# liayan/Legion-1

Hardware: AMD Instinct MI355X
Metric: sampled edges/s + feature GB/s, 3-hop GraphSAGE ogbn-papers100M at 1/2/4/8 GPU (higher is better)
Workload: dtype int32 ids / f32 rows (verbatim copy)

## Files before the change

### legion-1_amd/csrc/internal.h

```cpp
#pragma once
#include <hip/hip_runtime.h>
#include <cstdint>
#include <cstdio>
#include <cstdlib>
#include <iostream>
#include <string>
#include <vector>

#include "../../include/legion_amd.h"
#include "audit.h"

namespace legion {

void report_error(const char* file, int line, const char* msg, bool hip_failure);
bool error_pending();
bool error_is_fatal();
int64_t ipc_max_bytes();
bool ipc_size_ok(int64_t bytes, const char* who);
bool ipc_export_ok(const void* ptr, const char* who);
int64_t shard_chunk_bytes();
inline void check(hipError_t e, const char* file, int line)
{
    if (e != hipSuccess) report_error(file, line, hipGetErrorString(e), true);
}
#define HIP_CHECK(expr) ::legion::check((expr), __FILE__, __LINE__)
#define HIP_CHECK_LAST() ::legion::check(hipGetLastError(), __FILE__, __LINE__)
#define LEGION_ARG_ERROR(msg) ::legion::report_error(__FILE__, __LINE__, (msg), false)

std::ostream& log_out();
FILE* log_file();

int physical_device(int logical);
bool is_remote_device(int logical);
struct DeviceGuard {
    int prev = -1, prev_logical = -1;
    explicit DeviceGuard(int logical);
    ~DeviceGuard();
};

int chunk_shift(int64_t unit_bytes, int min_shift);
inline int chunk_count(int64_t n, int shift) { return n > 0 ? (int)(((n - 1) >> shift) + 1) : 1; }
template <typename T>
struct ChunkList {
    std::vector<T*> chunks;
    bool imported = false;
    T* at(int q) const { return q >= 0 && q < (int)chunks.size() ? chunks[q] : nullptr; }
    bool complete(size_t n) const { for (T* p : chunks) if (!p) return false; return chunks.size() == n; }
    void release();
    int export_chunk(int dev, int q, void* handle64, const char* who) const;
    int import_chunk(int q, const void* handle64, int64_t floor_bytes, int open_dev, const char* who);
};
template <typename T> void upload_table(int viewer, const std::vector<T*>& h, T**& tab, bool realloc, const char* what);

typedef unsigned long long pos_t;
constexpr int kPosShift = 32;
constexpr uint32_t kProvisional = 0x80000000u, kPosValueMask = 0x7FFFFFFFu;
constexpr uint32_t kEpochTop = 0xFFFFFFFFu, kSerialLimit = 0xFFFFFFF0u;
__host__ __device__ inline pos_t pos_entry(uint32_t epoch, uint32_t value) { return ((pos_t)epoch << kPosShift) | (pos_t)value; }
#ifndef LEGION_KTILE
#define LEGION_KTILE 1024
#endif
constexpr int kTile = LEGION_KTILE;
constexpr int kBlock = 256;
static_assert(kTile >= kBlock && kTile <= 2048 && (kTile & (kTile - 1)) == 0, "LEGION_KTILE: a power of two in [256, 2048] (k_sample stages 16 bytes of row descriptor per slot in static LDS)");
constexpr int kMaxChunks = 2048;
static_assert(kMaxChunks % kBlock == 0 && kMaxChunks >= 256 * 8, "kMaxChunks: a multiple of the workgroup size, >= 256 CUs x 8 workgroups");
constexpr int ilog2_c(int v) { return v <= 1 ? 0 : 1 + ilog2_c(v >> 1); }
constexpr int kMaxParts = LEGION_MAX_DEVICE;

constexpr uint32_t kP31 = 2147483647u;
constexpr uint32_t kA = 48271u;

__host__ __device__ inline uint32_t mulmod31(uint32_t a, uint32_t b)
{
    uint64_t p = (uint64_t)a * (uint64_t)b;
    uint32_t r = (uint32_t)(p & kP31) + (uint32_t)(p >> 31);
    r = (r & kP31) + (r >> 31);
    return r >= kP31 ? r - kP31 : r;
}

__host__ __device__ inline uint32_t powmod31(uint32_t base, uint64_t e)
{
    uint32_t r = 1;
    while (e) {
        if (e & 1) r = mulmod31(r, base);
        base = mulmod31(base, base);
        e >>= 1;
    }
    return r;
}

struct FastDiv {
    uint32_t d = 1, m = 0, s = 0;
    FastDiv() = default;
    explicit FastDiv(uint32_t div);
};

struct CsrTables {
    const int64_t* indptr;
    const int32_t* indices;
    const int64_t* const* frag_indptr;
    const int32_t* const* frag_indices;
    int32_t ip_nch, ix_nch, row_shift, edge_shift;
    int32_t partition_count;
    const int8_t* topo_owner;
    const int32_t* topo_row;
};

struct BatchCtl {
    int32_t counter;
    uint32_t epoch;
};

struct HopState {
    int32_t edge_base, node_base, n_edges, n_nodes, in_off, n_in, slots, pad;
};

struct SamplerBuffers {
    int32_t* sampled_ids;
    int32_t* agg_src_ids;
    int32_t* agg_src_off;
    int32_t* agg_dst_off;
    int32_t* nc;
    int32_t* ec;
    pos_t* pos_map;
    const BatchCtl* ctl;
    int32_t* cand;
    int32_t* aux;
    int32_t* aux_next;
    int32_t next_count;
    int32_t aux_cap;
    int32_t ids_cap;
    int32_t V;
    bool aux_prepared;
    int32_t* tile_edge;
    int32_t* tile_node;
    int2* tile_pre;
    int2* chunk_tot;
    HopState* hop_state;
    unsigned long long* edge_access_time;
};

void launch_seed(hipStream_t s, int32_t* batch_ids, int32_t* labels, int32_t batch_size, int32_t size, int32_t counter,
                 const int32_t* all_ids, const int32_t* all_labels, int32_t total_cap, pos_t* pos_map,
                 uint32_t epoch, BatchCtl* ctl, bool self_driven, int32_t* nc, int32_t* ec, int32_t* aux_next,
                 int32_t f_next, int32_t aux_cap);
void launch_set_cursor(hipStream_t s, BatchCtl* ctl, int32_t counter, uint32_t epoch);
void launch_advance(hipStream_t s, BatchCtl* ctl);
void warm_static_tables();
void launch_sample_hop(hipStream_t s, const CsrTables& csr, const SamplerBuffers& b, int32_t count, int32_t op_id,
                       int32_t hops, int32_t slots_bound, bool is_presc);
void launch_find_feat(hipStream_t s, const int32_t* sampled_ids, int32_t* cache_offset, const int32_t* nc,
                      int32_t op_id, const int32_t* feat_map, int32_t bound);
void launch_find_topo(hipStream_t s, const int32_t* input_ids, int8_t* part_index, int32_t* part_offset,
                      int32_t batch_size, const int8_t* topo_owner, const int32_t* topo_row);
struct GatherArgs {
    const float* table;
    const float* const* shard_tab;
    int32_t chunk_shift, nchunks;
    const int32_t* feat_map;
    const float** row_ptr;
    int32_t cache_capacity;
    int32_t F;
    int32_t table_pitch, shard_pitch;
    int32_t total_num_nodes;
    const int32_t* sampled_ids;
    const int32_t* nc;
    float* dst;
// ... 156 lines not shown
```

### legion-1_amd/csrc/kernels.hip

```cpp
#include "internal.h"
#include <hipcub/hipcub.hpp>
#include <mutex>
#include <cstring>

#include "audit_hooks.h"

namespace legion {

__device__ inline int32_t sample_index(uint32_t x, int32_t deg)
{
    double result = (double)(uint32_t)(x - 1u);
    result /= 2147483646.0;
    return (int32_t)(result * (double)deg + 0.0);
}

__device__ inline uint32_t fdiv(uint32_t n, const FastDiv& d)
{
    return d.d == 1 ? n : (uint32_t)(((uint64_t)n * d.m) >> d.s);
}

__device__ inline int lane_id() { return threadIdx.x & 63; }
__device__ inline int wave_id() { return threadIdx.x >> 6; }

__device__ inline int32_t total_nodes(const int32_t* nc, int32_t hops) { return nc[5 + 2 * hops]; }

template <bool SELF>
__global__ __launch_bounds__(kBlock) void k_seed(int32_t* __restrict__ batch_ids, int32_t* __restrict__ labels,
                                                 int32_t batch_size, int32_t size, int32_t counter,
                                                 const int32_t* __restrict__ all_ids,
                                                 const int32_t* __restrict__ all_labels, int32_t total_cap,
                                                 pos_t* __restrict__ pos_map, uint32_t epoch,
                                                 BatchCtl* __restrict__ ctl, int32_t* __restrict__ nc,
                                                 int32_t* __restrict__ ec, int32_t* __restrict__ aux_next,
                                                 int32_t f_next, int32_t aux_cap)
{
    int32_t idx = threadIdx.x + blockDim.x * blockIdx.x;
    if (SELF) {
        counter = ctl->counter;
        epoch = ctl->epoch;
        const int64_t done = (int64_t)batch_size * counter;
        size = (done + batch_size >= total_cap) ? (int32_t)max((int64_t)0, min((int64_t)batch_size, (int64_t)total_cap - done)) : batch_size;
    } else if (idx == 0) {
        ctl->counter = counter;
        ctl->epoch = epoch;
    }
    if (idx < size) {
        int32_t g = size * counter + idx;
        if (g >= total_cap) {
            batch_ids[idx] = -1;
            labels[idx] = -1;
        } else {
            int32_t src_id = all_ids[g % total_cap];
            batch_ids[idx] = src_id;
            const pos_t mine = pos_entry(epoch, (uint32_t)idx);
            pos_t cur = pos_map[src_id];
            while ((uint32_t)(cur >> kPosShift) != epoch || cur < mine) {
                const pos_t seen = atomicCAS(pos_map + src_id, cur, mine);
                if (seen == cur) break;
                cur = seen;
            }
            labels[idx] = all_labels[g % total_cap];
        }
    }
    if (idx < 16) {
        int32_t nv = 0;
        if (idx == 0 || idx == 2 || idx == 4) nv = size;
        nc[idx] = nv;
        ec[idx] = 0;
    }
    const int64_t n_init = min((int64_t)max(size, 0) * f_next, (int64_t)aux_cap);
    for (int64_t i = idx; i < n_init; i += (int64_t)gridDim.x * blockDim.x) aux_next[i] = -1;
}
__global__ void k_fill_aux(const int32_t* __restrict__ nc, int32_t count, int32_t* __restrict__ aux, int32_t aux_cap)
{
    const int64_t n = min((int64_t)nc[2] * count, (int64_t)aux_cap);
    for (int64_t i = threadIdx.x + (int64_t)blockDim.x * blockIdx.x; i < n; i += (int64_t)gridDim.x * blockDim.x) aux[i] = -1;
}
__global__ void k_set_cursor(BatchCtl* ctl, int32_t counter, uint32_t epoch) { ctl->counter = counter; ctl->epoch = epoch; }
__global__ void k_advance(BatchCtl* ctl) { ctl->counter += 1; ctl->epoch -= 1; }


struct SampleArgs {
    CsrTables csr;
    const int32_t* sampled_ids;
    const int32_t* agg_src_ids;
    const int32_t* nc;
    const int32_t* ec;
    pos_t* pos_map;
    int32_t* cand;
    int32_t* aux;
    int32_t* tile_edge;
    unsigned long long* edge_access_time;
    const BatchCtl* ctl;
    const uint32_t* pow_tab;
    uint32_t a_tile;
    uint32_t a_step;
    FastDiv fdiv;
    int32_t count;
    int32_t op_id;
    int32_t window;
    int32_t prefilter_from_op;
};

__device__ inline int32_t claim_slot(const SampleArgs& a, uint32_t epoch, int32_t dst, int32_t idx)
{
    const pos_t prov0 = pos_entry(epoch, kProvisional);
    const pos_t mine = prov0 | (pos_t)(uint32_t)idx;
    pos_t cur = (a.op_id < a.prefilter_from_op) ? ~(pos_t)0 : a.pos_map[dst];
    if (cur > mine) {
        const pos_t old = atomicMin(a.pos_map + dst, mine);
        if (old > mine) {
            if ((uint32_t)(old >> kPosShift) == epoch) a.aux[(uint32_t)old & kPosValueMask] = -2 - idx;
            cur = mine;
        } else {
            cur = old;
        }
    }
    if (cur < prov0) return (int32_t)((uint32_t)cur & kPosValueMask);
    if (cur < mine) return -2 - (int32_t)((uint32_t)cur & kPosValueMask);
    return -1;
}

template <bool PRESC, bool PARTITIONED>
__global__ __launch_bounds__(kBlock) void k_sample(SampleArgs a)
{
    __shared__ const int32_t* s_row[kTile + 2];
    __shared__ int32_t s_deg[kTile + 2];
    __shared__ int32_t s_src[kTile + 2];
    __shared__ int32_t s_cnt[kBlock / 64];

    const int32_t N = a.nc[2];
    const int32_t f = a.count;
    const int32_t total = N * f;
    const int32_t* __restrict__ input = (a.op_id == 2) ? a.sampled_ids : a.agg_src_ids + a.ec[2];
    const int32_t n_tiles = (total + kTile - 1) / kTile;
    const int tid = threadIdx.x;
    const uint32_t epoch = a.ctl->epoch;

    if ((int32_t)blockIdx.x >= n_tiles) return;

    uint32_t x[kTile / kBlock];
    {
        uint32_t base = powmod31(a.a_tile, (uint64_t)blockIdx.x);
#pragma unroll
        for (int s = 0; s < kTile / kBlock; s++) x[s] = mulmod31(base, a.pow_tab[tid + kBlock * s]);
    }

    for (int32_t tile = blockIdx.x; tile < n_tiles; tile += gridDim.x) {
        const int32_t tile_start = tile * kTile;
        const int32_t tile_end = min(tile_start + kTile, total);
        const int32_t i0 = (int32_t)fdiv((uint32_t)tile_start, a.fdiv);
        const int32_t i_last = (int32_t)fdiv((uint32_t)(tile_end - 1), a.fdiv);
        const int32_t nrows = i_last - i0 + 1;

        for (int32_t r = tid; r < nrows; r += kBlock) {
            const int32_t src = input[i0 + r];
            const int32_t* rowp = nullptr;
            int32_t deg = -1;
            if (src >= 0) {
                const int64_t* ip = a.csr.indptr + src;
                const int32_t* ix = a.csr.indices;
                int8_t owner = -1;
                if (PARTITIONED && !PRESC) owner = a.csr.topo_owner[src];
                if (owner >= 0) {
                    const int32_t row = a.csr.topo_row[src];
                    ip = a.csr.frag_indptr[owner * a.csr.ip_nch + (row >> a.csr.row_shift)] + (row & ((1 << a.csr.row_shift) - 1));
                    const int64_t start = ip[0];
                    ix = a.csr.frag_indices[owner * a.csr.ix_nch + (int32_t)(start >> a.csr.edge_shift)];
                    rowp = ix + (start & ((1ll << a.csr.edge_shift) - 1));
                    deg = (int32_t)(ip[1] - start);
                } else {
                    const int64_t start = ip[0];
                    rowp = ix + start;
                    deg = (int32_t)(ip[1] - start);
                }
            }
            s_row[r] = rowp;
            s_deg[r] = deg;
            s_src[r] = src;
        }
        __syncthreads();

        int32_t cnt = 0;
#pragma unroll
        for (int s = 0; s < kTile / kBlock; s++) {
            const int32_t idx = tile_start + tid + kBlock * s;
            int32_t dst = -1, known = -1, j = 0, r = 0;
            if (idx < tile_end) {
                const uint32_t i = fdiv((uint32_t)idx, a.fdiv);
                j = idx - (int32_t)i * f;
                r = (int32_t)i - i0;
                const int32_t deg = s_deg[r];
                if (j < deg) {
                    dst = s_row[r][sample_index(x[s], deg)];
                    if (dst < 0) dst = -1;
                }
            }
            int32_t dup = 0;
            for (int d = 1; d <= a.window; d++) {
                const int32_t o = __shfl_up(dst, d);
                if (d <= j && d <= lane_id() && o == dst) dup = d;
            }
            if (dst >= 0) {
                if (PRESC) atomicAdd(a.edge_access_time + s_src[r], 1ull);
                if (dup) known = -2 - (idx - dup);
                else known = claim_slot(a, epoch, dst, idx);
                cnt++;
            }
            if (idx < tile_end) {
                a.cand[idx] = dst;
                if (dst < 0) a.aux[idx] = 0;
                else if (known != -1) a.aux[idx] = known;
            }
        }
        for (int o = 32; o > 0; o >>= 1) cnt += __shfl_down(cnt, o);
        if (lane_id() == 0) s_cnt[wave_id()] = cnt;
        __syncthreads();
        if (tid == 0) {
            int32_t t = 0;
#pragma unroll
            for (int w = 0; w < kBlock / 64; w++) t += s_cnt[w];
            a.tile_edge[tile] = t;
        }
#pragma unroll
        for (int s = 0; s < kTile / kBlock; s++) x[s] = mulmod31(x[s], a.a_step);
        __syncthreads();
    }
}

constexpr int32_t kWinBase = 0x40000000;

__device__ inline int32_t enc_win(int32_t r) { return -2 - (kWinBase + r); }
__device__ inline bool is_win(int32_t v) { return v <= -2 - kWinBase; }
__device__ inline int32_t win_rank(int32_t v) { return -2 - v - kWinBase; }

__host__ __device__ inline FastDiv make_fastdiv(uint32_t div)
{
    FastDiv f;
    f.d = div ? div : 1;
    if (f.d == 1) { f.m = 0; f.s = 0; return f; }
    uint32_t l = 0;
    while ((1ull << l) < f.d) l++;
    f.m = (uint32_t)(((1ull << (31 + l)) / f.d) + 1ull);
    f.s = 31 + l;
    return f;
}

__global__ __launch_bounds__(kBlock) void k_mark(const int32_t* __restrict__ nc, const int32_t* __restrict__ ec,
                                                 int32_t count, int32_t* __restrict__ aux, const int32_t* __restrict__ tile_edge,
                                                 int32_t* __restrict__ tile_node, int2* __restrict__ tile_pre,
                                                 int2* __restrict__ chunk_tot, HopState* __restrict__ hs)
{
    constexpr int S = kTile / kBlock, W = kBlock / 64;
    __shared__ int32_t s_c[S * W];
    const int32_t total = nc[2] * count;
    const int32_t n_tiles = (total + kTile - 1) / kTile;
    const int lane = lane_id(), wave = wave_id();
    const unsigned long long lt = (1ull << lane) - 1ull;
    if (blockIdx.x == 0 && threadIdx.x == 0) {
        HopState h;
        h.edge_base = ec[0]; h.node_base = nc[0]; h.n_edges = 0; h.n_nodes = 0;
        h.in_off = ec[2]; h.n_in = nc[2]; h.slots = total; h.pad = 0;
        *hs = h;
    }
    const int32_t T = (n_tiles + (int32_t)gridDim.x - 1) / (int32_t)gridDim.x;
    const int32_t t0 = (int32_t)blockIdx.x * T, t1 = min(t0 + T, n_tiles);
    if (t0 >= n_tiles) return;
    int32_t nxt[S];
#pragma unroll
    for (int s = 0; s < S; s++) {
        const int64_t idx = (int64_t)t0 * kTile + threadIdx.x + kBlock * s;
        nxt[s] = idx < total ? aux[idx] : 0;
    }
    int32_t te_next = threadIdx.x == 0 ? tile_edge[t0] : 0, run_e = 0, run_n = 0;
    for (int32_t tile = t0; tile < t1; tile++) {
        bool win[S];
        int32_t rk[S];
        const int32_t te = te_next;
#pragma unroll
        for (int s = 0; s < S; s++) {
            const int32_t idx = tile * kTile + threadIdx.x + kBlock * s;
            win[s] = idx < total && nxt[s] == -1;
        }
        {
            const int64_t nt = (int64_t)tile + 1;
#pragma unroll
            for (int s = 0; s < S; s++) {
                const int64_t idx = nt * kTile + threadIdx.x + kBlock * s;
                nxt[s] = (nt < t1 && idx < total) ? aux[idx] : 0;
            }
            if (threadIdx.x == 0 && nt < t1) te_next = tile_edge[nt];
        }
#pragma unroll
        for (int s = 0; s < S; s++) {
            const unsigned long long b = __ballot(win[s]);
            rk[s] = __popcll(b & lt);
            if (lane == 0) s_c[s * W + wave] = __popcll(b);
        }
        __syncthreads();
        int32_t run = 0, before[S];
#pragma unroll
        for (int q = 0; q < S * W; q++) {
#pragma unroll
            for (int s = 0; s < S; s++)
                if (q == s * W + wave) before[s] = run;
            run += s_c[q];
        }
#pragma unroll
        for (int s = 0; s < S; s++)
            if (win[s]) aux[tile * kTile + threadIdx.x + kBlock * s] = enc_win(before[s] + rk[s]);
        if (threadIdx.x == 0) {
            tile_node[tile] = run;
            tile_pre[tile] = make_int2(run_e, run_n);
            run_e += te; run_n += run;
        }
        __syncthreads();
    }
    if (threadIdx.x == 0) chunk_tot[blockIdx.x] = make_int2(run_e, run_n);
}

__device__ inline void apply_update_counter(int32_t* nc, int32_t* ec, int32_t op_id, int32_t hops, int32_t n_nodes,
                                            int32_t n_edges)
{
    const int32_t hh = op_id / 2;
    nc[0] += n_nodes;
    nc[3 + 2 * hh] = nc[1 + 2 * hh] + nc[2 + 2 * hh];
    nc[4 + 2 * hh] = n_nodes;
    if (hh == hops) nc[5 + 2 * hh] = nc[3 + 2 * hh] + nc[4 + 2 * hh];
    nc[1] = 0;
    nc[2] = n_edges;
    ec[2 + hh] = (hh == 1 ? ec[3] : ec[1 + hh]) + n_edges;
    ec[2] = ec[0];
    ec[0] += n_edges;
    ec[1] = 0;
}

struct WriteArgs {
    HopState* hs;
    int32_t* nc;
    int32_t* ec;
    int32_t hops;
    const int32_t* cand;
    const int32_t* aux;
    const int32_t* tile_edge;
    const int32_t* tile_node;
    int32_t* sampled_ids;
    int32_t* agg_src_ids;
    int32_t* agg_src_off;
    int32_t* agg_dst_off;
    pos_t* pos_map;
    FastDiv fdiv;
    int32_t op_id;
    const BatchCtl* ctl;
    int32_t last_hop;
    const int2* tile_pre;
    const int2* chunk_tot;
    int32_t mark_grid;
    int32_t* aux_next;
    int32_t next_count;
    int32_t aux_cap;
    int32_t ids_cap;
    int32_t V;
};

#define LEGION_STORE_OK(i, cap) ((uint32_t)(i) < (uint32_t)(cap))

__global__ __launch_bounds__(kBlock) void k_write(WriteArgs a)
{
    constexpr int S = kTile / kBlock, W = kBlock / 64;
    __shared__ int2 s_chunk[kMaxChunks];
    __shared__ int32_t s_e[S * W];
    __shared__ int2 s_scan[W];
    __shared__ uint32_t s_div_t[3];
    const HopState h = *a.hs;
    const uint32_t epoch = a.ctl->epoch;
    const int32_t total = h.slots;
    const int32_t n_tiles = (total + kTile - 1) / kTile;
    const int lane = lane_id(), wave = wave_id();
    const unsigned long long lt = (1ull << lane) - 1ull;
    if (n_tiles == 0) {
        if (blockIdx.x == 0 && threadIdx.x == 0) apply_update_counter(a.nc, a.ec, a.op_id, a.hops, 0, 0);
        return;
    }
    if ((int32_t)blockIdx.x >= n_tiles) return;
    const int32_t T = (n_tiles + a.mark_grid - 1) / a.mark_grid;
    if (threadIdx.x == 0) {
        const FastDiv f = make_fastdiv((uint32_t)T);
        s_div_t[0] = f.d; s_div_t[1] = f.m; s_div_t[2] = f.s;
    }
    const int32_t n_chunks = (n_tiles + T - 1) / T;
    {
        constexpr int PER = kMaxChunks / kBlock;
        const int32_t q0 = (int32_t)threadIdx.x * PER;
        int2 v[PER];
#pragma unroll
        for (int u = 0; u < PER; u++) v[u] = a.chunk_tot[min(q0 + u, n_chunks - 1)];
        int32_t se = 0, sn = 0;
#pragma unroll
        for (int u = 0; u < PER; u++) {
            if (q0 + u >= n_chunks) v[u] = make_int2(0, 0);
            se += v[u].x; sn += v[u].y;
        }
        int32_t ie = se, in = sn;
        for (int o = 1; o < 64; o <<= 1) {
            const int32_t ue = __shfl_up(ie, o), un = __shfl_up(in, o);
            if (lane >= o) { ie += ue; in += un; }
        }
        if (lane == 63) s_scan[wave] = make_int2(ie, in);
// ... 3 lines not shown
        for (int w = 0; w < W; w++)
            if (w < wave) { run_e += s_scan[w].x; run_n += s_scan[w].y; }
#pragma unroll
        for (int u = 0; u < PER; u++) {
            if (q0 + u < n_chunks) s_chunk[q0 + u] = make_int2(run_e, run_n);
            run_e += v[u].x; run_n += v[u].y;
        }
        __syncthreads();
    }
    FastDiv div_t;
    div_t.d = s_div_t[0]; div_t.m = s_div_t[1]; div_t.s = s_div_t[2];
    auto nodes_before = [&](int32_t t, int32_t pre_n_in_chunk) { return s_chunk[fdiv((uint32_t)t, div_t)].y + pre_n_in_chunk; };

    for (int32_t tile = blockIdx.x; tile < n_tiles; tile += gridDim.x) {
        const int2 own = a.tile_pre[tile], own_chunk = s_chunk[fdiv((uint32_t)tile, div_t)];
        const int32_t pre_e = own_chunk.x + own.x, pre_n = own_chunk.y + own.y;
        const int32_t tile_e = a.tile_edge[tile];
        const int32_t ebase = h.edge_base + pre_e;
        const int32_t nbase = h.node_base + pre_n;
        int32_t c[S], so[S], dpos[S], w[S], re[S], wpre[S];
        const int32_t* __restrict__ pre_n_of = reinterpret_cast<const int32_t*>(a.tile_pre) + 1;
#pragma unroll
        for (int s = 0; s < S; s++) {
            const int32_t idx = tile * kTile + threadIdx.x + kBlock * s;
            c[s] = (idx < total) ? a.cand[idx] : -1;
            so[s] = (idx < total) ? a.aux[idx] : 0;
        }
#pragma unroll
        for (int s = 0; s < S; s++) {
            dpos[s] = 0; w[s] = -1;
            if (c[s] == -1) continue;
            const int32_t idx = tile * kTile + threadIdx.x + kBlock * s;
            const int32_t i = (int32_t)fdiv((uint32_t)idx, a.fdiv);
            dpos[s] = (a.op_id == 2) ? (int32_t)((uint32_t)a.pos_map[a.sampled_ids[i]] & kPosValueMask) : a.agg_src_off[h.in_off + i];
            wpre[s] = 0;
            if (so[s] < -1 && !is_win(so[s])) { w[s] = -2 - so[s]; so[s] = a.aux[w[s]]; wpre[s] = pre_n_of[2 * (w[s] / kTile)]; }
        }
#pragma unroll
        for (int s = 0; s < S; s++)
            while (w[s] >= 0 && so[s] < -1 && !is_win(so[s])) { w[s] = -2 - so[s]; so[s] = a.aux[w[s]]; wpre[s] = pre_n_of[2 * (w[s] / kTile)]; }
#pragma unroll
        for (int s = 0; s < S; s++) {
            const unsigned long long be = __ballot(c[s] != -1);
            re[s] = __popcll(be & lt);
            if (lane == 0) s_e[s * W + wave] = __popcll(be);
        }
        __syncthreads();
        if (tile == n_tiles - 1 && threadIdx.x == 0) {
            const int32_t n_edges = pre_e + tile_e, n_nodes = pre_n + a.tile_node[tile];
            a.hs->n_edges = n_edges;
            a.hs->n_nodes = n_nodes;
            apply_update_counter(a.nc, a.ec, a.op_id, a.hops, n_nodes, n_edges);
        }
#pragma unroll
        for (int s = 0; s < S; s++) {
            if (c[s] == -1) continue;
            int32_t pe = 0;
            for (int q = 0; q < s * W + wave; q++) pe += s_e[q];
            const int32_t dst = c[s];
            const int32_t e = ebase + pe + re[s];
            if (!LEGION_STORE_OK(e, a.ids_cap)) continue;
            if (!a.last_hop) a.agg_src_ids[e] = dst;
            a.agg_dst_off[e] = dpos[s];
            int32_t p = so[s];
            if (w[s] >= 0) {
                if (p < -1)
                    p = h.node_base + nodes_before(w[s] / kTile, wpre[s]) + win_rank(p);
// ... 469 lines not shown
void launch_seed(hipStream_t s, int32_t* batch_ids, int32_t* labels, int32_t batch_size, int32_t size, int32_t counter,
                 const int32_t* all_ids, const int32_t* all_labels, int32_t total_cap, pos_t* pos_map,
                 uint32_t epoch, BatchCtl* ctl, bool self_driven, int32_t* nc, int32_t* ec, int32_t* aux_next,
                 int32_t f_next, int32_t aux_cap)
{
    const int32_t bound = self_driven ? batch_size : size;
    int blocks = bound > 0 ? (bound - 1) / kBlock + 1 : 1;
    LEGION_AUDIT_LAUNCH(s, "k_seed", LEGION_AW(batch_ids), LEGION_AW(labels), LEGION_AW(pos_map), LEGION_AW(ctl), LEGION_AW(nc), LEGION_AW(ec), LEGION_AW(aux_next), LEGION_AL(all_ids), LEGION_AL(all_labels));
    if (self_driven) k_seed<true><<<blocks, kBlock, 0, s>>>(batch_ids, labels, batch_size, size, counter, all_ids, all_labels, total_cap, pos_map, epoch, ctl, nc, ec, aux_next, f_next, aux_cap);
    else k_seed<false><<<blocks, kBlock, 0, s>>>(batch_ids, labels, batch_size, size, counter, all_ids, all_labels, total_cap, pos_map, epoch, ctl, nc, ec, aux_next, f_next, aux_cap);
    HIP_CHECK_LAST();
}
void launch_set_cursor(hipStream_t s, BatchCtl* ctl, int32_t counter, uint32_t epoch)
{
    LEGION_AUDIT_LAUNCH(s, "k_set_cursor", LEGION_AW(ctl));
    k_set_cursor<<<1, 1, 0, s>>>(ctl, counter, epoch);
    HIP_CHECK_LAST();
}
void launch_advance(hipStream_t s, BatchCtl* ctl)
{
    LEGION_AUDIT_LAUNCH(s, "k_advance", LEGION_AW(ctl));
    k_advance<<<1, 1, 0, s>>>(ctl);
    HIP_CHECK_LAST();
}
void warm_static_tables() { (void)pow_table(); (void)cu_count(); }

void launch_sample_hop(hipStream_t s, const CsrTables& csr, const SamplerBuffers& b, int32_t count, int32_t op_id,
                       int32_t hops, int32_t slots_bound, bool is_presc)
{
    if (count <= 0 || slots_bound <= 0) { LEGION_ARG_ERROR("GPU_Random_Sampling: empty hop"); return; }
    const int max_tiles = (slots_bound + kTile - 1) / kTile;
    constexpr int wg_per_cu = 4;
    const int grid = std::min(grid_for(max_tiles, 1, wg_per_cu), kMaxChunks);
    if (!b.aux_prepared) {
        LEGION_AUDIT_LAUNCH(s, "k_fill_aux", LEGION_AW(b.aux), LEGION_AL(b.nc));
        k_fill_aux<<<grid_for(slots_bound, kBlock * 4), kBlock, 0, s>>>(b.nc, count, b.aux, b.aux_cap);
        HIP_CHECK_LAST();
    }
    SampleArgs a;
    a.csr = csr;
    a.sampled_ids = b.sampled_ids; a.agg_src_ids = b.agg_src_ids; a.nc = b.nc; a.ec = b.ec;
    a.pos_map = b.pos_map; a.cand = b.cand; a.aux = b.aux; a.tile_edge = b.tile_edge;
    a.edge_access_time = b.edge_access_time;
    a.ctl = b.ctl;
    a.pow_tab = pow_table();
    a.a_tile = powmod31(kA, kTile);
    a.a_step = powmod31(kA, (uint64_t)kTile * (uint64_t)grid);
    a.fdiv = FastDiv((uint32_t)count);
    a.count = count; a.op_id = op_id;
    a.window = std::min(count - 1, 8);
    a.prefilter_from_op = 4;
    const bool part = csr.topo_owner != nullptr;
    LEGION_AUDIT_LAUNCH(s, "k_sample", LEGION_AW(a.pos_map), LEGION_AW(a.cand), LEGION_AW(a.aux), LEGION_AW(a.tile_edge), LEGION_AW(a.edge_access_time), LEGION_AL(a.sampled_ids), LEGION_AL(a.agg_src_ids), LEGION_AL(a.nc), LEGION_AL(a.ec), LEGION_AL(a.ctl), LEGION_AL(a.pow_tab), LEGION_AL(csr.frag_indptr), LEGION_AL(csr.frag_indices), LEGION_AL(csr.topo_owner), LEGION_AL(csr.topo_row), LEGION_AR(csr.indptr), LEGION_AR(csr.indices));
    if (is_presc) k_sample<true, false><<<grid, kBlock, 0, s>>>(a);
    else if (part) k_sample<false, true><<<grid, kBlock, 0, s>>>(a);
    else k_sample<false, false><<<grid, kBlock, 0, s>>>(a);
    HIP_CHECK_LAST();
    LEGION_AUDIT_LAUNCH(s, "k_mark", LEGION_AW(b.aux), LEGION_AW(b.tile_node), LEGION_AW(b.tile_pre), LEGION_AW(b.chunk_tot), LEGION_AW(b.hop_state), LEGION_AL(b.nc), LEGION_AL(b.ec), LEGION_AL(b.tile_edge));
    k_mark<<<grid, kBlock, 0, s>>>(b.nc, b.ec, count, b.aux, b.tile_edge, b.tile_node, b.tile_pre, b.chunk_tot, b.hop_state);
    HIP_CHECK_LAST();
    WriteArgs w;
    w.hs = b.hop_state; w.nc = b.nc; w.ec = b.ec; w.hops = hops; w.cand = b.cand; w.aux = b.aux; w.ctl = b.ctl; w.tile_edge = b.tile_edge; w.tile_node = b.tile_node;
    w.sampled_ids = b.sampled_ids; w.agg_src_ids = b.agg_src_ids; w.agg_src_off = b.agg_src_off;
    w.agg_dst_off = b.agg_dst_off; w.pos_map = b.pos_map; w.fdiv = a.fdiv; w.op_id = op_id; w.last_hop = (op_id / 2 == hops) ? 1 : 0;
    w.aux_next = b.aux_next; w.next_count = b.next_count; w.aux_cap = b.aux_cap; w.ids_cap = b.ids_cap; w.V = b.V;
    w.tile_pre = b.tile_pre; w.chunk_tot = b.chunk_tot; w.mark_grid = grid;
    const int wgrid = grid_for(max_tiles, 1, 8);
    LEGION_AUDIT_LAUNCH(s, "k_write", LEGION_AW(w.hs), LEGION_AW(w.nc), LEGION_AW(w.ec), LEGION_AW(w.sampled_ids), LEGION_AW(w.agg_src_ids), LEGION_AW(w.agg_src_off), LEGION_AW(w.agg_dst_off), LEGION_AW(w.pos_map), LEGION_AW(w.aux_next), LEGION_AL(w.cand), LEGION_AL(w.aux), LEGION_AL(w.tile_edge), LEGION_AL(w.tile_node), LEGION_AL(w.tile_pre), LEGION_AL(w.chunk_tot), LEGION_AL(w.ctl));
    k_write<<<wgrid, kBlock, 0, s>>>(w);
    HIP_CHECK_LAST();
}

void launch_find_feat(hipStream_t s, const int32_t* sampled_ids, int32_t* cache_offset, const int32_t* nc,
                      int32_t op_id, const int32_t* feat_map, int32_t bound)
{
    const int l = (op_id - 1) / 2;
    LEGION_AUDIT_LAUNCH(s, "k_find_feat", LEGION_AW(cache_offset), LEGION_AL(sampled_ids), LEGION_AL(nc), LEGION_AL(feat_map));
    k_find_feat<<<grid_for(bound, kBlock), kBlock, 0, s>>>(sampled_ids, cache_offset, nc, 3 + 2 * l, 4 + 2 * l, feat_map);
    HIP_CHECK_LAST();
}

void launch_find_topo(hipStream_t s, const int32_t* input_ids, int8_t* part_index, int32_t* part_offset,
                      int32_t batch_size, const int8_t* topo_owner, const int32_t* topo_row)
{
    if (batch_size <= 0) return;
    LEGION_AUDIT_LAUNCH(s, "k_find_topo", LEGION_AW(part_index), LEGION_AW(part_offset), LEGION_AL(input_ids), LEGION_AL(topo_owner), LEGION_AL(topo_row));
    k_find_topo<<<grid_for(batch_size, kBlock), kBlock, 0, s>>>(input_ids, part_index, part_offset, batch_size, topo_owner, topo_row);
    HIP_CHECK_LAST();
}

void launch_gather(hipStream_t s, const GatherArgs& g, int32_t rows_bound)
{
// ... 223 lines not shown
```

### legion-1_amd/csrc/launchers.cpp

```cpp
#include "internal.h"

#include <cstring>
#include <iostream>

#include "audit_hooks.h"

using namespace legion;

static inline int pool_dev(const GPUMemoryPool* p)
{
    if (p->device_id >= 0) return p->device_id;
    if (current_logical_device() >= 0) return current_logical_device();
    int d = 0;
    (void)hipGetDevice(&d);
    return d;
}

static bool pool_ready(const GPUMemoryPool* p, const char* who)
{
    if (!p || !p->owns_scratch) { LEGION_ARG_ERROR((std::string(who) + ": GPUMemoryPool_AllocateScratch was not called").c_str()); return false; }
    const int q = p->current_pipe;
    if (!p->sampled_ids[q] || !p->labels[q] || !p->agg_src_off[q] || !p->agg_dst_off[q] || !p->node_counter[q] || !p->edge_counter[q]) {
        LEGION_ARG_ERROR((std::string(who) + ": output buffers of the current pipe are not set").c_str());
        return false;
// ... 63 lines not shown
                p->ctl, false, p->node_counter[q], p->edge_counter[q], p->aux2[1], p->fanout[0], p->max_slots);
    p->aux_ready_hop = 1; p->aux_ready_count = p->fanout[0];
    p->bound_n = size > 0 ? size : 0;
    p->bound_nodes = p->bound_n;
}

void GPU_Random_Sampling(void* strm_hdl, GPUGraphStorage* graph, GPUCache* cache, GPUMemoryPool* memorypool,
                         int32_t count, int32_t op_id, int is_presc)
{
    if (graph == nullptr) { log_out() << "invalid storage ptr\n"; return; }
    if (!pool_ready(memorypool, "GPU_Random_Sampling")) return;
    GPUMemoryPool* p = memorypool;
    const int hop = op_id / 2;
    if (op_id < 2 || (op_id & 1) || hop > p->hops) { LEGION_ARG_ERROR("GPU_Random_Sampling: op_id must be 2,4,..,2*hops"); return; }
    const int dev = pool_dev(p);
    const int P = graph->partition_count;
    if (dev < 0 || dev >= P) { LEGION_ARG_ERROR("GPU_Random_Sampling: device outside the partition table"); return; }
    const int64_t slots = (int64_t)p->bound_n * count;
    if (slots > p->max_slots) { LEGION_ARG_ERROR("GPU_Random_Sampling: fan-out exceeds what the pool was sized for"); return; }
    if (slots <= 0) return;

    CsrTables csr;
    csr.partition_count = P;
    csr.indptr = graph->replica_indptr[dev] ? graph->replica_indptr[dev] : graph->csr_node_index_cpu;
    csr.indices = graph->replica_indices[dev] ? graph->replica_indices[dev] : graph->csr_dst_node_ids_cpu;
    csr.frag_indptr = nullptr; csr.frag_indices = nullptr;
    csr.ip_nch = csr.ix_nch = 1; csr.row_shift = graph->row_shift; csr.edge_shift = graph->edge_shift;
    csr.topo_owner = nullptr;
    csr.topo_row = nullptr;
    SamplerBuffers b;
    const int q = p->current_pipe;
    b.sampled_ids = p->sampled_ids[q]; b.agg_src_ids = p->agg_src_ids; b.agg_src_off = p->agg_src_off[q];
    b.agg_dst_off = p->agg_dst_off[q]; b.nc = p->node_counter[q]; b.ec = p->edge_counter[q];
    b.pos_map = p->pos_map; b.ctl = p->ctl; b.cand = p->cand; b.aux = p->aux2[hop & 1]; b.aux_next = p->aux2[(hop + 1) & 1]; b.tile_edge = p->tile_edge; b.tile_node = p->tile_node; b.tile_pre = p->tile_pre; b.chunk_tot = p->chunk_tot;
    b.hop_state = p->hop_state; b.edge_access_time = nullptr;
    if (is_presc) {
        if (!cache || dev >= cache->device_count || !cache->ctl[dev]->edge_access_time) { LEGION_ARG_ERROR("GPU_Random_Sampling: pre-sampling needs an initialised cache controller"); return; }
        b.edge_access_time = cache->ctl[dev]->edge_access_time;
    } else if (cache && dev < cache->device_count && cache->ctl[dev]->topo_owner && cache->ctl[dev]->edge_capacity > 0) {
        bool all = graph->d_frag_tab[dev] != nullptr;
        const int Kg = cache->Kg, K0 = (dev / Kg) * Kg;
        for (int g = K0; g < K0 + Kg && all; g++) all = graph->view[dev][g] && graph->frag[g].complete;
        if (all) {
            csr.frag_indptr = (const int64_t* const*)graph->d_frag_tab[dev];
            csr.frag_indices = (const int32_t* const*)(graph->d_frag_tab[dev] + (size_t)P * graph->ip_nch);
            csr.ip_nch = graph->ip_nch; csr.ix_nch = graph->ix_nch;
            csr.topo_owner = cache->ctl[dev]->topo_owner; csr.topo_row = cache->ctl[dev]->topo_row;
        }
    }
    b.aux_cap = p->max_slots;
    b.ids_cap = p->num_ids;
    b.V = p->V;
    b.aux_prepared = p->aux_ready_hop == hop && p->aux_ready_count == count;
    b.next_count = hop < p->hops ? p->fanout[hop] : 0;
    launch_sample_hop((hipStream_t)strm_hdl, csr, b, count, op_id, p->hops, (int32_t)slots, is_presc != 0);
    p->aux_ready_hop = hop + 1; p->aux_ready_count = b.next_count;
    p->bound_n = (int32_t)slots;
    p->bound_nodes += (int32_t)slots;
}

static bool gather_args(GatherArgs& g, GPUCache* cache, GPUNodeStorage* noder, GPUMemoryPool* p, int32_t dev_id, int off_idx, int size_idx,
                        bool count_hits = true)
{
    const int32_t F = noder->float_attr_len;
    if (F < 0) log_out() << "error feature len\n";
    const int q = p->current_pipe;
    if (!p->float_features[q]) { LEGION_ARG_ERROR("get_feature_kernel: feature buffer of the current pipe is not set"); return false; }
// ... 238 lines not shown
```

### legion-1_amd/csrc/runtime.cpp

```cpp
#include "internal.h"

#include <cstring>
#include <mutex>

#include "audit_hooks.h"

namespace legion {

static int g_error_mode = LEGION_ERR_EXIT;
static thread_local std::string t_last_error;
static int g_dev_map[64];
static bool g_dev_map_set[64];
static std::mutex g_mu;
static bool g_remote[64];

void report_error(const char* file, int line, const char* msg, bool hip_failure)
{
    char buf[1024];
    snprintf(buf, sizeof(buf), "%s failure %s:%d: '%s'", hip_failure ? "Hip" : "Legion", file, line, msg);
    if (hip_failure && g_error_mode == LEGION_ERR_EXIT) {
        fprintf(log_file(), "%s\n", buf);
        fflush(log_file());
        exit(EXIT_FAILURE);
    }
    if (t_last_error.empty()) t_last_error = buf;
    if (!hip_failure && g_error_mode == LEGION_ERR_EXIT) fprintf(stderr, "%s\n", buf);
    (void)hipGetLastError();
}

static int log_to_stderr()
{
    static const int v = [] { const char* e = getenv("LEGION_LOG"); return (e && strcmp(e, "stderr") == 0) ? 1 : 0; }();
    return v;
}
std::ostream& log_out() { return log_to_stderr() ? std::cerr : std::cout; }
FILE* log_file() { return log_to_stderr() ? stderr : stdout; }

bool error_pending() { return !t_last_error.empty(); }
bool error_is_fatal() { return g_error_mode == LEGION_ERR_EXIT; }

int64_t ipc_max_bytes()
{
    const char* e = getenv("LEGION_IPC_MAX_BYTES");
    return e && atoll(e) > 0 ? atoll(e) : LEGION_IPC_MAX_BYTES_DEFAULT;
}
int64_t shard_chunk_bytes()
{
    const char* e = getenv("LEGION_SHARD_CHUNK_BYTES");
    return e && atoll(e) > 0 ? atoll(e) : (1ll << 30);
}
bool ipc_size_ok(int64_t bytes, const char* who)
{
    if (bytes <= ipc_max_bytes()) return true;
    char msg[320];
    snprintf(msg, sizeof(msg), "%s: a single allocation of %lld bytes exceeds the HIP-IPC limit of %lld bytes (LEGION_IPC_MAX_BYTES): "
             "larger single allocations never finish importing on this driver; use the chunked calls / a smaller buffer",
             who, (long long)bytes, (long long)ipc_max_bytes());
    report_error(__FILE__, __LINE__, msg, false);
    return false;
}
bool ipc_export_ok(const void* ptr, const char* who)
{
    hipDeviceptr_t base = nullptr;
    size_t size = 0;
    if (hipMemGetAddressRange(&base, &size, (hipDeviceptr_t)ptr) != hipSuccess) { (void)hipGetLastError(); return true; }
    return ipc_size_ok((int64_t)size, who);
}

bool is_remote_device(int logical) { return logical >= 0 && logical < 64 && g_remote[logical]; }

int physical_device(int logical)
{
    if (logical >= 0 && logical < 64 && g_dev_map_set[logical]) return g_dev_map[logical];
    int n = 0;
    if (hipGetDeviceCount(&n) != hipSuccess || n <= 0) return 0;
    return logical >= 0 ? logical % n : 0;
}

DeviceGuard::DeviceGuard(int logical)
{
    HIP_CHECK(hipGetDevice(&prev));
    int want = physical_device(logical);
    if (want != prev) HIP_CHECK(hipSetDevice(want));
// ... 143 lines not shown
```

### legion-1_amd/csrc/storage.cpp

```cpp
#include "internal.h"

#include <algorithm>
#include <cstring>
#include <set>

#include "audit_hooks.h"

using namespace legion;

static void enable_p2p(int32_t partition_count)
{
    std::set<int> phys;
    for (int i = 0; i < partition_count; i++) phys.insert(physical_device(i));
    if (audit::on()) for (int a = 0; a < partition_count; a++) for (int b = 0; b < partition_count; b++) if (a != b) audit::record_peer(a, b);
    if (phys.size() < 2) return;
    int cur = 0;
    HIP_CHECK(hipGetDevice(&cur));
    for (int a : phys) {
        HIP_CHECK(hipSetDevice(a));
        for (int b : phys) {
            if (a == b) continue;
            int ok = 0;
            HIP_CHECK(hipDeviceCanAccessPeer(&ok, a, b));
            if (ok) {
// ... 407 lines not shown
    agg_src_off.assign(pipeline_depth, nullptr);
    agg_dst_off.assign(pipeline_depth, nullptr);
}

extern "C" {

GPUMemoryPool* NewGPUMemoryPool(int32_t pipeline_depth) { return new GPUMemoryPool(pipeline_depth); }

void GPUMemoryPool_AllocateScratch(GPUMemoryPool* p, int32_t total_num_nodes, int32_t batch_size,
                                   const int32_t* fanout, int32_t hops)
{
    if (!p || hops < 1 || hops > LEGION_MAX_HOPS || batch_size < 1 || total_num_nodes < 1) { LEGION_ARG_ERROR("GPUMemoryPool_AllocateScratch: bad arguments"); return; }
    if (p->owns_scratch) GPUMemoryPool_Finalize(p);
    p->V = total_num_nodes; p->batch_size = batch_size; p->hops = hops;
    int64_t ids = batch_size, cur = batch_size, max_slots = 0;
    p->level_bound[0] = batch_size;
    for (int h = 0; h < hops; h++) {
        p->fanout[h] = fanout[h];
        cur *= fanout[h];
        if (cur > max_slots) max_slots = cur;
        ids += cur;
        if (ids >= (1ll << 31)) { LEGION_ARG_ERROR("GPUMemoryPool_AllocateScratch: batch*fanouts exceeds int32"); return; }
        if (cur >= (1ll << 30)) { LEGION_ARG_ERROR("GPUMemoryPool_AllocateScratch: a hop of 2^30 or more slots exceeds the slot-state encoding"); return; }
        p->level_bound[h + 1] = (int32_t)cur;
    }
    p->num_ids = (int32_t)ids;
    p->max_slots = (int32_t)max_slots;
    p->max_tiles = (int32_t)((max_slots + kTile - 1) / kTile);
    p->owns_scratch = true;
    HIP_CHECK(hipMalloc(&p->pos_map, (size_t)total_num_nodes * sizeof(pos_t)));
    HIP_CHECK(hipMemset(p->pos_map, 0xFF, (size_t)total_num_nodes * sizeof(pos_t)));
    p->batch_serial = 0;
    HIP_CHECK(hipMalloc(&p->ctl, sizeof(BatchCtl)));
    { const BatchCtl c{0, kEpochTop}; HIP_CHECK(hipMemcpy(p->ctl, &c, sizeof(c), hipMemcpyHostToDevice)); }
    p->ctl_synced = false;
    HIP_CHECK(hipHostMalloc((void**)&p->rows_seen, (LEGION_MAX_HOPS + 2) * sizeof(int32_t), hipHostMallocMapped));
    memset(p->rows_seen, 0, (LEGION_MAX_HOPS + 2) * sizeof(int32_t));
    HIP_CHECK(hipHostGetDevicePointer((void**)&p->rows_seen_dev, p->rows_seen, 0));
    HIP_CHECK(hipMalloc(&p->cand, (size_t)p->max_slots * sizeof(int32_t)));
    for (auto& a : p->aux2) HIP_CHECK(hipMalloc(&a, (size_t)p->max_slots * sizeof(int32_t)));
    HIP_CHECK(hipMalloc(&p->tile_edge, (size_t)(p->max_tiles + 1) * sizeof(int32_t)));
    HIP_CHECK(hipMalloc(&p->tile_node, (size_t)(p->max_tiles + 1) * sizeof(int32_t)));
    HIP_CHECK(hipMalloc(&p->tile_pre, (size_t)(p->max_tiles + 1) * sizeof(int2)));
    HIP_CHECK(hipMalloc(&p->chunk_tot, (size_t)kMaxChunks * sizeof(int2)));
    HIP_CHECK(hipMalloc(&p->hop_state, sizeof(HopState)));
    HIP_CHECK(hipMalloc(&p->cache_search_buffer, (size_t)p->num_ids * sizeof(int32_t)));
    HIP_CHECK(hipMalloc((void**)&p->row_ptr, (size_t)p->num_ids * sizeof(float*)));
    HIP_CHECK(hipMalloc(&p->agg_src_ids, (size_t)p->num_ids * sizeof(int32_t)));
    HIP_CHECK(hipMalloc(&p->tmp_part_ind, (size_t)p->num_ids));
    HIP_CHECK(hipMalloc(&p->tmp_part_off, (size_t)p->num_ids * sizeof(int32_t)));
    HIP_CHECK(hipDeviceSynchronize());
}
int32_t GPUMemoryPool_NumIds(const GPUMemoryPool* p) { return p->num_ids; }

#define POOL_PIPE_SETTER(name, field, type) \
    void GPUMemoryPool_Set##name(GPUMemoryPool* p, type* ptr, int32_t pipe) { \
        if (pipe < 0 || pipe >= p->pipeline_depth) { LEGION_ARG_ERROR("GPUMemoryPool_Set" #name ": bad pipe"); return; } \
        p->field[pipe] = ptr; } \
    type* GPUMemoryPool_Get##name(const GPUMemoryPool* p) { return p->field[p->current_pipe]; }
POOL_PIPE_SETTER(SampledIds, sampled_ids, int32_t)
POOL_PIPE_SETTER(FloatFeatures, float_features, float)
POOL_PIPE_SETTER(Labels, labels, int32_t)
POOL_PIPE_SETTER(AggSrcOf, agg_src_off, int32_t)
POOL_PIPE_SETTER(AggDstOf, agg_dst_off, int32_t)
POOL_PIPE_SETTER(NodeCounter, node_counter, int32_t)
POOL_PIPE_SETTER(EdgeCounter, edge_counter, int32_t)
#undef POOL_PIPE_SETTER
void GPUMemoryPool_SetFeatureRows(GPUMemoryPool* p, int32_t rows) { p->feature_rows = rows; }
void GPUMemoryPool_SetCurrentPipe(GPUMemoryPool* p, int32_t pipe) { p->current_pipe = pipe % p->pipeline_depth; }
void GPUMemoryPool_SetCurrentMode(GPUMemoryPool* p, int32_t mode) { p->mode = mode; }
void GPUMemoryPool_SetIter(GPUMemoryPool* p, int32_t iter) { p->iter = iter; }
int32_t GPUMemoryPool_GetCurrentMode(const GPUMemoryPool* p) { return p->mode; }
int32_t GPUMemoryPool_GetIter(const GPUMemoryPool* p) { return p->iter; }
int32_t* GPUMemoryPool_GetAggSrcId(const GPUMemoryPool* p) { return p->agg_src_ids; }
// ... 28 lines not shown
```

Before: 6.457 billion.

## Split k_sample tiles across multiple workgroups and skip seed pos_map lookups

When a hop has few tiles relative to CU capacity, k_sample now splits each tile's slots across up to four workgroups, each writing its own partial edge count that k_mark sums. This raises occupancy on small hops such as the first hop at small batch sizes. The cost is per-tile recomputation of the RNG base via powmod and a larger tile_edge buffer. Separately, the seed kernel records whether any duplicate seed ids occurred, and the first hop skips the pos_map gather when there were none, using the slot index directly.

```diff
diff --git a/legion-1_amd/csrc/internal.h b/legion-1_amd/csrc/internal.h
--- a/legion-1_amd/csrc/internal.h
+++ b/legion-1_amd/csrc/internal.h
@@ -19,6 +19,7 @@
 bool ipc_size_ok(int64_t bytes, const char* who);
 bool ipc_export_ok(const void* ptr, const char* who);
 int64_t shard_chunk_bytes();
+int sample_split_mode();
 inline void check(hipError_t e, const char* file, int line)
 {
     if (e != hipSuccess) report_error(file, line, hipGetErrorString(e), true);
@@ -65,6 +66,8 @@
 static_assert(kTile >= kBlock && kTile <= 2048 && (kTile & (kTile - 1)) == 0, "LEGION_KTILE: a power of two in [256, 2048] (k_sample stages 16 bytes of row descriptor per slot in static LDS)");
 constexpr int kMaxChunks = 2048;
 static_assert(kMaxChunks % kBlock == 0 && kMaxChunks >= 256 * 8, "kMaxChunks: a multiple of the workgroup size, >= 256 CUs x 8 workgroups");
+constexpr int kMaxSplit = 4;
+constexpr int kSplitCap = (kTile / kBlock) < kMaxSplit ? (kTile / kBlock) : kMaxSplit;
 constexpr int ilog2_c(int v) { return v <= 1 ? 0 : 1 + ilog2_c(v >> 1); }
 constexpr int kMaxParts = LEGION_MAX_DEVICE;
 
@@ -110,6 +113,7 @@
 struct BatchCtl {
     int32_t counter;
     uint32_t epoch;
+    uint32_t dup_epoch;
 };
 
 struct HopState {
@@ -134,6 +138,7 @@
     int32_t V;
     bool aux_prepared;
     int32_t* tile_edge;
+    int32_t tile_stride;
     int32_t* tile_node;
     int2* tile_pre;
     int2* chunk_tot;
diff --git a/legion-1_amd/csrc/kernels.hip b/legion-1_amd/csrc/kernels.hip
--- a/legion-1_amd/csrc/kernels.hip
+++ b/legion-1_amd/csrc/kernels.hip
@@ -54,11 +54,14 @@
             batch_ids[idx] = src_id;
             const pos_t mine = pos_entry(epoch, (uint32_t)idx);
             pos_t cur = pos_map[src_id];
+            bool dup = (uint32_t)(cur >> kPosShift) == epoch;
             while ((uint32_t)(cur >> kPosShift) != epoch || cur < mine) {
                 const pos_t seen = atomicCAS(pos_map + src_id, cur, mine);
                 if (seen == cur) break;
                 cur = seen;
+                dup |= (uint32_t)(cur >> kPosShift) == epoch;
             }
+            if (dup) ctl->dup_epoch = epoch;
             labels[idx] = all_labels[g % total_cap];
         }
     }
@@ -90,6 +93,8 @@
     int32_t* cand;
     int32_t* aux;
     int32_t* tile_edge;
+    int32_t tile_stride;
+    int32_t split_shift;
     unsigned long long* edge_access_time;
     const BatchCtl* ctl;
     const uint32_t* pow_tab;
@@ -137,21 +142,31 @@
     const int tid = threadIdx.x;
     const uint32_t epoch = a.ctl->epoch;
 
-    if ((int32_t)blockIdx.x >= n_tiles) return;
+    const int32_t g = (int32_t)blockIdx.x & ((1 << a.split_shift) - 1);
+    const int32_t tile0 = (int32_t)blockIdx.x >> a.split_shift, tile_step = (int32_t)gridDim.x >> a.split_shift;
+    const int s_lo = g * ((kTile / kBlock) >> a.split_shift), s_hi = s_lo + ((kTile / kBlock) >> a.split_shift);
+    if (tile0 >= n_tiles) return;
 
     uint32_t x[kTile / kBlock];
-    {
-        uint32_t base = powmod31(a.a_tile, (uint64_t)blockIdx.x);
+    if (a.split_shift == 0) {
+        uint32_t base = powmod31(a.a_tile, (uint64_t)tile0);
 #pragma unroll
         for (int s = 0; s < kTile / kBlock; s++) x[s] = mulmod31(base, a.pow_tab[tid + kBlock * s]);
     }
 
-    for (int32_t tile = blockIdx.x; tile < n_tiles; tile += gridDim.x) {
+    for (int32_t tile = tile0; tile < n_tiles; tile += tile_step) {
+        if (a.split_shift != 0) {
+            const uint32_t base = powmod31(a.a_tile, (uint64_t)tile);
+#pragma unroll
+            for (int s = 0; s < kTile / kBlock; s++)
+                if (s >= s_lo && s < s_hi) x[s] = mulmod31(base, a.pow_tab[tid + kBlock * s]);
+        }
         const int32_t tile_start = tile * kTile;
         const int32_t tile_end = min(tile_start + kTile, total);
-        const int32_t i0 = (int32_t)fdiv((uint32_t)tile_start, a.fdiv);
-        const int32_t i_last = (int32_t)fdiv((uint32_t)(tile_end - 1), a.fdiv);
-        const int32_t nrows = i_last - i0 + 1;
+        const int32_t sub_start = tile_start + kBlock * s_lo;
+        const int32_t sub_end = min(tile_start + kBlock * s_hi, tile_end);
+        const int32_t i0 = (int32_t)fdiv((uint32_t)min(sub_start, tile_end - 1), a.fdiv);
+        const int32_t nrows = sub_end > sub_start ? (int32_t)fdiv((uint32_t)(sub_end - 1), a.fdiv) - i0 + 1 : 0;
 
         for (int32_t r = tid; r < nrows; r += kBlock) {
             const int32_t src = input[i0 + r];
@@ -184,6 +199,7 @@
         int32_t cnt = 0;
 #pragma unroll
         for (int s = 0; s < kTile / kBlock; s++) {
+            if (s < s_lo || s >= s_hi) continue;
             const int32_t idx = tile_start + tid + kBlock * s;
             int32_t dst = -1, known = -1, j = 0, r = 0;
             if (idx < tile_end) {
@@ -220,10 +236,12 @@
             int32_t t = 0;
 #pragma unroll
             for (int w = 0; w < kBlock / 64; w++) t += s_cnt[w];
-            a.tile_edge[tile] = t;
-        }
-#pragma unroll
-        for (int s = 0; s < kTile / kBlock; s++) x[s] = mulmod31(x[s], a.a_step);
+            a.tile_edge[g * a.tile_stride + tile] = t;
+        }
+        if (a.split_shift == 0) {
+#pragma unroll
+            for (int s = 0; s < kTile / kBlock; s++) x[s] = mulmod31(x[s], a.a_step);
+        }
         __syncthreads();
     }
 }
@@ -247,10 +265,16 @@
 }
 
 __global__ __launch_bounds__(kBlock) void k_mark(const int32_t* __restrict__ nc, const int32_t* __restrict__ ec,
-                                                 int32_t count, int32_t* __restrict__ aux, const int32_t* __restrict__ tile_edge,
+                                                 int32_t count, int32_t* __restrict__ aux, int32_t* __restrict__ tile_edge,
+                                                 int32_t split, int32_t tile_stride,
                                                  int32_t* __restrict__ tile_node, int2* __restrict__ tile_pre,
                                                  int2* __restrict__ chunk_tot, HopState* __restrict__ hs)
 {
+    auto edges_of = [&](int32_t t) {
+        int32_t e = tile_edge[t];
+        for (int32_t g = 1; g < split; g++) e += tile_edge[g * tile_stride + t];
+        return e;
+    };
     constexpr int S = kTile / kBlock, W = kBlock / 64;
     __shared__ int32_t s_c[S * W];
     const int32_t total = nc[2] * count;
@@ -272,7 +296,7 @@
         const int64_t idx = (int64_t)t0 * kTile + threadIdx.x + kBlock * s;
         nxt[s] = idx < total ? aux[idx] : 0;
     }
-    int32_t te_next = threadIdx.x == 0 ? tile_edge[t0] : 0, run_e = 0, run_n = 0;
+    int32_t te_next = threadIdx.x == 0 ? edges_of(t0) : 0, run_e = 0, run_n = 0;
     for (int32_t tile = t0; tile < t1; tile++) {
         bool win[S];
         int32_t rk[S];
@@ -289,7 +313,7 @@
                 const int64_t idx = nt * kTile + threadIdx.x + kBlock * s;
                 nxt[s] = (nt < t1 && idx < total) ? aux[idx] : 0;
             }
-            if (threadIdx.x == 0 && nt < t1) te_next = tile_edge[nt];
+            if (threadIdx.x == 0 && nt < t1) te_next = edges_of((int32_t)nt);
         }
 #pragma unroll
         for (int s = 0; s < S; s++) {
@@ -311,6 +335,7 @@
             if (win[s]) aux[tile * kTile + threadIdx.x + kBlock * s] = enc_win(before[s] + rk[s]);
         if (threadIdx.x == 0) {
             tile_node[tile] = run;
+            if (split > 1) tile_edge[tile] = te;
             tile_pre[tile] = make_int2(run_e, run_n);
             run_e += te; run_n += run;
         }
@@ -374,6 +399,7 @@
     __shared__ uint32_t s_div_t[3];
     const HopState h = *a.hs;
     const uint32_t epoch = a.ctl->epoch;
+    const bool seed_lookup = a.op_id == 2 && a.ctl->dup_epoch == epoch;
     const int32_t total = h.slots;
     const int32_t n_tiles = (total + kTile - 1) / kTile;
     const int lane = lane_id(), wave = wave_id();
@@ -443,7 +469,8 @@
             if (c[s] == -1) continue;
             const int32_t idx = tile * kTile + threadIdx.x + kBlock * s;
             const int32_t i = (int32_t)fdiv((uint32_t)idx, a.fdiv);
-            dpos[s] = (a.op_id == 2) ? (int32_t)((uint32_t)a.pos_map[a.sampled_ids[i]] & kPosValueMask) : a.agg_src_off[h.in_off + i];
+            if (a.op_id != 2) dpos[s] = a.agg_src_off[h.in_off + i];
+            else dpos[s] = seed_lookup ? (int32_t)((uint32_t)a.pos_map[a.sampled_ids[i]] & kPosValueMask) : i;
             wpre[s] = 0;
             if (so[s] < -1 && !is_win(so[s])) { w[s] = -2 - so[s]; so[s] = a.aux[w[s]]; wpre[s] = pre_n_of[2 * (w[s] / kTile)]; }
         }
@@ -979,6 +1006,13 @@
     const int max_tiles = (slots_bound + kTile - 1) / kTile;
     constexpr int wg_per_cu = 4;
     const int grid = std::min(grid_for(max_tiles, 1, wg_per_cu), kMaxChunks);
+    const int forced = sample_split_mode();
+    int split = 1;
+    if (forced > 0) split = std::min(forced, kSplitCap);
+    else
+        for (int g = kSplitCap; g > 1 && split == 1; g >>= 1)
+            if ((int64_t)max_tiles * g <= (int64_t)cu_count() * wg_per_cu) split = g;
+    const int sgrid = split == 1 ? grid : split * std::min(max_tiles, cu_count() * wg_per_cu / split);
     if (!b.aux_prepared) {
         LEGION_AUDIT_LAUNCH(s, "k_fill_aux", LEGION_AW(b.aux), LEGION_AL(b.nc));
         k_fill_aux<<<grid_for(slots_bound, kBlock * 4), kBlock, 0, s>>>(b.nc, count, b.aux, b.aux_cap);
@@ -987,7 +1021,9 @@
     SampleArgs a;
     a.csr = csr;
     a.sampled_ids = b.sampled_ids; a.agg_src_ids = b.agg_src_ids; a.nc = b.nc; a.ec = b.ec;
-    a.pos_map = b.pos_map; a.cand = b.cand; a.aux = b.aux; a.tile_edge = b.tile_edge;
+    a.pos_map = b.pos_map; a.cand = b.cand; a.aux = b.aux;
+    a.tile_edge = b.tile_edge;
+    a.tile_stride = b.tile_stride; a.split_shift = ilog2_c(split);
     a.edge_access_time = b.edge_access_time;
     a.ctl = b.ctl;
     a.pow_tab = pow_table();
@@ -999,12 +1035,12 @@
     a.prefilter_from_op = 4;
     const bool part = csr.topo_owner != nullptr;
     LEGION_AUDIT_LAUNCH(s, "k_sample", LEGION_AW(a.pos_map), LEGION_AW(a.cand), LEGION_AW(a.aux), LEGION_AW(a.tile_edge), LEGION_AW(a.edge_access_time), LEGION_AL(a.sampled_ids), LEGION_AL(a.agg_src_ids), LEGION_AL(a.nc), LEGION_AL(a.ec), LEGION_AL(a.ctl), LEGION_AL(a.pow_tab), LEGION_AL(csr.frag_indptr), LEGION_AL(csr.frag_indices), LEGION_AL(csr.topo_owner), LEGION_AL(csr.topo_row), LEGION_AR(csr.indptr), LEGION_AR(csr.indices));
-    if (is_presc) k_sample<true, false><<<grid, kBlock, 0, s>>>(a);
-    else if (part) k_sample<false, true><<<grid, kBlock, 0, s>>>(a);
-    else k_sample<false, false><<<grid, kBlock, 0, s>>>(a);
+    if (is_presc) k_sample<true, false><<<sgrid, kBlock, 0, s>>>(a);
+    else if (part) k_sample<false, true><<<sgrid, kBlock, 0, s>>>(a);
+    else k_sample<false, false><<<sgrid, kBlock, 0, s>>>(a);
     HIP_CHECK_LAST();
     LEGION_AUDIT_LAUNCH(s, "k_mark", LEGION_AW(b.aux), LEGION_AW(b.tile_node), LEGION_AW(b.tile_pre), LEGION_AW(b.chunk_tot), LEGION_AW(b.hop_state), LEGION_AL(b.nc), LEGION_AL(b.ec), LEGION_AL(b.tile_edge));
-    k_mark<<<grid, kBlock, 0, s>>>(b.nc, b.ec, count, b.aux, b.tile_edge, b.tile_node, b.tile_pre, b.chunk_tot, b.hop_state);
+    k_mark<<<grid, kBlock, 0, s>>>(b.nc, b.ec, count, b.aux, b.tile_edge, split, b.tile_stride, b.tile_node, b.tile_pre, b.chunk_tot, b.hop_state);
     HIP_CHECK_LAST();
     WriteArgs w;
     w.hs = b.hop_state; w.nc = b.nc; w.ec = b.ec; w.hops = hops; w.cand = b.cand; w.aux = b.aux; w.ctl = b.ctl; w.tile_edge = b.tile_edge; w.tile_node = b.tile_node;
diff --git a/legion-1_amd/csrc/launchers.cpp b/legion-1_amd/csrc/launchers.cpp
--- a/legion-1_amd/csrc/launchers.cpp
+++ b/legion-1_amd/csrc/launchers.cpp
@@ -119,7 +119,7 @@
     const int q = p->current_pipe;
     b.sampled_ids = p->sampled_ids[q]; b.agg_src_ids = p->agg_src_ids; b.agg_src_off = p->agg_src_off[q];
     b.agg_dst_off = p->agg_dst_off[q]; b.nc = p->node_counter[q]; b.ec = p->edge_counter[q];
-    b.pos_map = p->pos_map; b.ctl = p->ctl; b.cand = p->cand; b.aux = p->aux2[hop & 1]; b.aux_next = p->aux2[(hop + 1) & 1]; b.tile_edge = p->tile_edge; b.tile_node = p->tile_node; b.tile_pre = p->tile_pre; b.chunk_tot = p->chunk_tot;
+    b.pos_map = p->pos_map; b.ctl = p->ctl; b.cand = p->cand; b.aux = p->aux2[hop & 1]; b.aux_next = p->aux2[(hop + 1) & 1]; b.tile_edge = p->tile_edge; b.tile_stride = p->max_tiles + 1; b.tile_node = p->tile_node; b.tile_pre = p->tile_pre; b.chunk_tot = p->chunk_tot;
     b.hop_state = p->hop_state; b.edge_access_time = nullptr;
     if (is_presc) {
         if (!cache || dev >= cache->device_count || !cache->ctl[dev]->edge_access_time) { LEGION_ARG_ERROR("GPU_Random_Sampling: pre-sampling needs an initialised cache controller"); return; }
diff --git a/legion-1_amd/csrc/runtime.cpp b/legion-1_amd/csrc/runtime.cpp
--- a/legion-1_amd/csrc/runtime.cpp
+++ b/legion-1_amd/csrc/runtime.cpp
@@ -49,6 +49,14 @@
     const char* e = getenv("LEGION_SHARD_CHUNK_BYTES");
     return e && atoll(e) > 0 ? atoll(e) : (1ll << 30);
 }
+int sample_split_mode()
+{
+    const char* e = getenv("LEGION_SAMPLE_SPLIT");
+    if (!e || !e[0] || strcmp(e, "auto") == 0) return 0;
+    if (strcmp(e, "off") == 0) return 1;
+    const int v = atoi(e);
+    return (v == 1 || v == 2 || v == 4) ? v : 0;
+}
 bool ipc_size_ok(int64_t bytes, const char* who)
 {
     if (bytes <= ipc_max_bytes()) return true;
diff --git a/legion-1_amd/csrc/storage.cpp b/legion-1_amd/csrc/storage.cpp
--- a/legion-1_amd/csrc/storage.cpp
+++ b/legion-1_amd/csrc/storage.cpp
@@ -463,14 +463,14 @@
     HIP_CHECK(hipMemset(p->pos_map, 0xFF, (size_t)total_num_nodes * sizeof(pos_t)));
     p->batch_serial = 0;
     HIP_CHECK(hipMalloc(&p->ctl, sizeof(BatchCtl)));
-    { const BatchCtl c{0, kEpochTop}; HIP_CHECK(hipMemcpy(p->ctl, &c, sizeof(c), hipMemcpyHostToDevice)); }
+    { const BatchCtl c{0, kEpochTop, 0}; HIP_CHECK(hipMemcpy(p->ctl, &c, sizeof(c), hipMemcpyHostToDevice)); }
     p->ctl_synced = false;
     HIP_CHECK(hipHostMalloc((void**)&p->rows_seen, (LEGION_MAX_HOPS + 2) * sizeof(int32_t), hipHostMallocMapped));
     memset(p->rows_seen, 0, (LEGION_MAX_HOPS + 2) * sizeof(int32_t));
     HIP_CHECK(hipHostGetDevicePointer((void**)&p->rows_seen_dev, p->rows_seen, 0));
     HIP_CHECK(hipMalloc(&p->cand, (size_t)p->max_slots * sizeof(int32_t)));
     for (auto& a : p->aux2) HIP_CHECK(hipMalloc(&a, (size_t)p->max_slots * sizeof(int32_t)));
-    HIP_CHECK(hipMalloc(&p->tile_edge, (size_t)(p->max_tiles + 1) * sizeof(int32_t)));
+    HIP_CHECK(hipMalloc(&p->tile_edge, (size_t)kMaxSplit * (p->max_tiles + 1) * sizeof(int32_t)));
     HIP_CHECK(hipMalloc(&p->tile_node, (size_t)(p->max_tiles + 1) * sizeof(int32_t)));
     HIP_CHECK(hipMalloc(&p->tile_pre, (size_t)(p->max_tiles + 1) * sizeof(int2)));
     HIP_CHECK(hipMalloc(&p->chunk_tot, (size_t)kMaxChunks * sizeof(int2)));
```

Result: no change. 6.513 billion, median of 6 (+0.9%).
